# bcgsc/NanoSim

Hardware: AMD Instinct MI355X
Metric: simulated reads/sec (genome mode, mean 8 kb) (higher is better)
Workload: dtype u8

## Files before the change

nanosim_amd/csrc/nanosim_amd.hip:

```cpp
#include <hip/hip_runtime.h>
#include <hipcub/hipcub.hpp>
#include <stdio.h>
#include <stdlib.h>
#include <string.h>
#include <algorithm>
#include <chrono>
#include <atomic>
#include <condition_variable>
#include <functional>
#include <mutex>
#include <thread>
#include <type_traits>
#include <string>
#include <vector>

#include "ns_device.h"
#include "ns_materialise.h"
#include "ns_chain.h"
#include "ns_hp.h"
#include "ns_ir.h"
#include "ns_io.h"
#include "ns_pack.h"
#include "ns_cs_hist.h"
#include "ns_qual_hist.h"
// ... 950 lines not shown
                dst[L - 1 - (done + i)] = normalise_base(c);
            } else dst[done + i] = normalise_base(c);
        }
        done += end - start;
    });
    if (lane == 0) pp->ref_gpos = NS_SPLICED_BASE + off + NS_IR_PAD;
}

#ifndef NS_MAT_WAVES
#define NS_MAT_WAVES 7
#endif

__device__ __forceinline__ bool load_read_uniform(const GenArgs &A, uint64_t r, bool fastq, ns_read &rd, ns_key &key, ReadOut &ro) {
    rd = A.reads[r];
    if (rd.flags) return false;
    rd.rec_off = uni64(A.rec_off[r]);
    rd.piece_off = uni(rd.piece_off); rd.n_pieces = (uint16_t)uni(rd.n_pieces);
    rd.reversed = (uint8_t)uni(rd.reversed); rd.head = uni(rd.head); rd.tail = uni(rd.tail); rd.seq_len = uni(rd.seq_len);
    rd.attempts = uni(rd.attempts);
    key = read_key(A, r);
    key.r_lo = uni(key.r_lo); key.r_hi = uni(key.r_hi);
    ro.seq = A.records + rd.rec_off + uni(A.name_len[r]) + 2;
    ro.qual = fastq ? ro.seq + rd.seq_len + 3 : nullptr;
    ro.seq_len = rd.seq_len; ro.reversed = rd.reversed != 0; ro.uracil = A.prm.uracil != 0;
    return true;
}

#ifndef NS_MATQ_WAVES
#define NS_MATQ_WAVES 4
#endif
#ifndef NS_MATQ_MINW
#define NS_MATQ_MINW 6
#endif
__device__ __forceinline__ uint64_t hp_ev_slot(const GenArgs &A, uint64_t pos, uint32_t piece) { return (pos >> A.hp_shift) + (uint64_t)A.hp_pad * piece; }

#ifndef NS_TILE_CHUNKS_FINAL
#define NS_TILE_CHUNKS_FINAL 4u
#endif
#ifndef NS_MAT_WAVES_FINAL
#define NS_MAT_WAVES_FINAL 6
#endif
template <bool FASTQ, int MODE>
__global__ void __launch_bounds__(64, MODE == MAT_HP_FINAL ? NS_MAT_WAVES_FINAL : NS_MAT_WAVES)
k_materialise(GenArgs A, uint32_t dbg, SlowQueue sq, const uint32_t *order) {
    constexpr bool CLSOUT = FASTQ && MODE != MAT_HP_SCRATCH;
    constexpr uint32_t TC = MODE == MAT_HP_FINAL ? NS_TILE_CHUNKS_FINAL : NS_TILE_CHUNKS;
    __shared__ TileLds<TC> T;
    const uint32_t lane = threadIdx.x;
    const uint64_t slot = blockIdx.x;
    if (slot >= A.prm.n_reads) return;
    const uint64_t r = order ? (uint64_t)uni(order[slot]) : slot;
    ns_read rd; ns_key key; ReadOut ro;
    if (!load_read_uniform(A, r, false, rd, key, ro)) return;
    const uint32_t a = rd.attempts;
    tile_lds_init(T, lane);
    uint32_t *cls = nullptr;
    if constexpr (CLSOUT) cls = A.cls + cls_word0(rd.rec_off, r, cls_per_read(A.prm));
    if constexpr (MODE == MAT_HP_SCRATCH) {
        ro.seq = A.scr + uni64(A.scr_off[r]); ro.qual = nullptr; ro.reversed = false; ro.uracil = false;
        uint32_t q = 0;
        for (uint32_t pi = 0; pi < rd.n_pieces; ++pi) {
            const PieceCtx pc = load_piece_uniform(A.events, A.ref, A.pieces[rd.piece_off + pi], pi);
            materialise_piece<FASTQ, MODE, TC>(A.m, A.ref, T, ro, key, a, pc, q, lane, dbg, sq, (uint32_t)r, pi, nullptr);
            q += pc.out_len;
        }
        return;
    }
#ifdef NS_ABLATE
    if (!(dbg & 8))
#endif
    emit_head_tail(ro, key, a, rd.head, rd.tail, lane);
    uint32_t q = rd.head;
    uint64_t q_in = MODE == MAT_HP_FINAL ? uni64(A.scr_off[r]) : 0;
    for (uint32_t pi = 0; pi < rd.n_pieces; ++pi) {
        PieceCtx pc;
        if constexpr (MODE == MAT_HP_FINAL) {
            const uint32_t gp = rd.piece_off + pi;
            const ns_piece p = A.pieces[gp];
            const uint64_t eo = hp_ev_slot(A, q_in, uni(A.hp_pord[r]) + pi);
            pc.kind = uni(p.kind);
            pc.ev = A.hp_ev + eo; pc.wd = A.hp_wd + eo; pc.n_ev = pc.kind ? 0u : uni(A.hp_nev[gp]);
            pc.ref_len = uni(p.out_len); pc.out_len = pc.kind ? pc.ref_len : uni(A.hp_len[gp]);
            pc.chrom_base = (uint64_t)((uintptr_t)A.scr - (uintptr_t)A.ref.bases) + q_in; pc.chrom_len = ~0ull; pc.pos = 0;
            pc.sid = pc.kind ? NS_GAP_SEG + (pi >> 1) : (pi >> 1);
            q_in += pc.ref_len;
        } else pc = load_piece_uniform(A.events, A.ref, A.pieces[rd.piece_off + pi], pi);
        materialise_piece<FASTQ, MODE, TC>(A.m, A.ref, T, ro, key, a, pc, q, lane, dbg, sq, (uint32_t)r, pi, CLSOUT ? cls + (q >> 4) + 2u * pi : nullptr);
        q += pc.out_len;
    }
    if (A.polya) {
        const uint32_t pl = uni(A.polya[r]);
        if (pl) emit_polya(ro, q, pl, lane);
    }
}

template <bool HPF>
__global__ void __launch_bounds__(64 * NS_MATQ_WAVES, NS_MATQ_MINW) k_qualities(GenArgs A, const uint32_t *order) {
    __shared__ __align__(16) uint16_t qlut[NS_QLUT_SLOTS * 1024u];
    qual_lut_load(qlut, A.m, threadIdx.x, 64 * NS_MATQ_WAVES);
    __syncthreads();
    const uint32_t lane = threadIdx.x & 63u;
    const uint64_t slot = (uint64_t)blockIdx.x * NS_MATQ_WAVES + (threadIdx.x >> 6);
    if (slot >= A.prm.n_reads) return;
    const uint64_t r = order ? (uint64_t)uni(order[slot]) : slot;
    ns_read rd; ns_key key; ReadOut ro;
    if (!load_read_uniform(A, r, true, rd, key, ro)) return;
    const uint32_t a = rd.attempts;
    QualState Q; Q.lut = qlut;
    qualities_head_tail(A.m, Q, ro, key, a, rd.head, rd.tail, lane);
    const uint32_t *cls = A.cls + cls_word0(rd.rec_off, r, cls_per_read(A.prm));
    uint32_t q = rd.head;
    for (uint32_t pi = 0; pi < rd.n_pieces; ++pi) {
        const uint32_t gp = rd.piece_off + pi;
        const ns_piece p = A.pieces[gp];
        const uint32_t kind = uni(p.kind);
        const uint32_t out_len = (HPF && !kind) ? uni(A.hp_len[gp]) : uni(p.out_len);
        qualities_piece(A.m, Q, ro, key, a, kind ? NS_GAP_SEG + (pi >> 1) : (pi >> 1), kind, out_len, q, cls + (q >> 4) + 2u * pi, lane);
        q += out_len;
    }
    if (A.polya) {
        const uint32_t pl = uni(A.polya[r]);
        if (pl) emit_polya_quals(A.m, ro, key, a, q, pl, rd.head, rd.tail, lane);
    }
}

// ... 1205 lines not shown
        uint32_t *cnt = ctx->list_b.view<uint32_t>(), *seg_off = ctx->list_c.view<uint32_t>();
        k_dense_plan<<<dim3((unsigned)((n + 1 + 255) / 256)), dim3(256), 0, st>>>(A, cnt);
        HIPCHK(hipGetLastError());
        if (int rc = scan_sum(ctx, cnt, seg_off, n + 1)) return rc;
        const uint64_t bound = total_bases / NS_DENSE_SEG + n + 1;
        if (bound > 0x7fffffffull) return fail(ctx, NS_EINVAL, "unaligned batch too large for one launch of the record kernel (split it)");
        k_materialise_dense<<<dim3((unsigned)bound), dim3(64), 0, st>>>(A, seg_off);
        HIPCHK(hipGetLastError());
        if (fastq) {
            k_qualities<false><<<dim3((unsigned)((n + NS_MATQ_WAVES - 1) / NS_MATQ_WAVES)), dim3(64 * NS_MATQ_WAVES), 0, st>>>(A, nullptr);
            HIPCHK(hipGetLastError());
        }
        return NS_OK;
    }
    for (int round = 0;; ++round) {
        size_t cap = ctx->slow_q.cap >= 16 + sizeof(SlowTile) ? (ctx->slow_q.cap - 16) / sizeof(SlowTile) : 0;
        if (cap < n / 4 + 4096) {
            int rc = ensure(ctx, ctx->slow_q, 16 + (n / 4 + 4096) * sizeof(SlowTile));
            if (rc) return rc;
            cap = (ctx->slow_q.cap - 16) / sizeof(SlowTile);
            ctx->sq_zeroed = false;
        }
        SlowQueue sq;
        sq.count = ctx->slow_q.view<uint32_t>(); sq.items = ctx->slow_q.view<SlowTile>(16);
        sq.cap = (uint32_t)(cap > 0xffffffffull ? 0xffffffffull : cap);
        if (!(ctx->sq_zeroed && round == 0)) HIPCHK(hipMemsetAsync(sq.count, 0, 4, st));
        ctx->sq_zeroed = false;
        if (ctx->knob.dbg & 1024u) order = nullptr;
        const dim3 grid_q((unsigned)((n + NS_MATQ_WAVES - 1) / NS_MATQ_WAVES)), blk_q(64 * NS_MATQ_WAVES), grid_1((unsigned)n), blk_1(64);
        const uint32_t *order_b = (ctx->knob.dbg & 2048u) ? order : nullptr;
        if (round == 0) HIPCHK(hipEventRecord(ctx->evt[EV_RECKERNEL_BEGIN], st));
        by_fastq_mode(fastq, mode, [&](auto fq, auto md) {
            constexpr bool FQ = decltype(fq)::value; constexpr int MD = decltype(md)::value;
            k_materialise<FQ, MD><<<grid_1, blk_1, 0, st>>>(A, ctx->knob.dbg, sq, (MD == MAT_REF || (FQ && MD == MAT_HP_FINAL)) ? order_b : nullptr);
        });
        HIPCHK(hipGetLastError());
        if (round == 0) { HIPCHK(hipEventRecord(ctx->evt[EV_RECKERNEL_END], st)); ctx->rec_timed = true; }
        if (fastq && mode != MAT_HP_SCRATCH && round == 0) {
            if (mode == MAT_HP_FINAL) k_qualities<true><<<grid_q, blk_q, 0, st>>>(A, order);
            else k_qualities<false><<<grid_q, blk_q, 0, st>>>(A, order);
            HIPCHK(hipGetLastError());
        }
        uint32_t queued = 0;
        if (int rc2 = read_small(ctx, st, &queued, sq.count, 4)) return rc2;
        if (queued > sq.cap) {
            if (round >= 2) return fail(ctx, NS_ENOMEM, "slow-tile queue overflow");
            int rc = ensure(ctx, ctx->slow_q, 16 + ((size_t)queued + 4096) * sizeof(SlowTile));
            if (rc) return rc;
            continue;
        }
        if (queued) {
            const unsigned grid = queued < 16384u ? queued : 16384u;
            by_fastq_mode(fastq, mode, [&](auto fq, auto md) {
                constexpr bool FQ = decltype(fq)::value; constexpr int MD = decltype(md)::value;
                if constexpr (MD == MAT_HP_FINAL) k_materialise_slow_hpf<FQ><<<dim3(grid), dim3(64), 0, st>>>(A, sq);
                else k_materialise_slow<FQ, MD == MAT_HP_SCRATCH><<<dim3(grid), dim3(64), 0, st>>>(A, sq);
            });
            HIPCHK(hipGetLastError());
        }
        return NS_OK;
    }
}

static int hp_stage1(ns_ctx *ctx, const ns_params *prm, GenArgs &A, size_t n, uint64_t tot_pieces, unsigned long long *stats, double *ms_hp) {
    hipStream_t st = ctx->stream;
    const dim3 blk(256), grid_t((unsigned)((n + 1 + 255) / 256));
    int rc;
// ... 1858 lines not shown
```

nanosim_amd/csrc/ns_materialise.h:

```cpp
#pragma once
#include "ns_device.h"

#ifndef NS_TILE_CHUNKS
#define NS_TILE_CHUNKS 2u
#endif
#define T_EV 64u
#define NS_CLS_MIS_BIT 0x08u
#define NS_CLS_INS_BIT 0x20u
#define NS_CLS_STRIP 0xd7d7d7d7u
#define NS_QLUT_SLOTS 5u
__device__ __forceinline__ uint32_t wave_incl_scan(uint32_t v) {
    v += (uint32_t)__builtin_amdgcn_update_dpp(0, (int)v, 0x111, 0xf, 0xf, true);
    v += (uint32_t)__builtin_amdgcn_update_dpp(0, (int)v, 0x112, 0xf, 0xf, true);
    v += (uint32_t)__builtin_amdgcn_update_dpp(0, (int)v, 0x114, 0xf, 0xf, true);
    v += (uint32_t)__builtin_amdgcn_update_dpp(0, (int)v, 0x118, 0xf, 0xf, true);
    v += (uint32_t)__builtin_amdgcn_update_dpp(0, (int)v, 0x142, 0xa, 0xf, false);
    v += (uint32_t)__builtin_amdgcn_update_dpp(0, (int)v, 0x143, 0xc, 0xf, false);
    return v;
}

__device__ __forceinline__ uint32_t wave_incl_max(uint32_t v) {
    v = max(v, (uint32_t)__builtin_amdgcn_update_dpp(0, (int)v, 0x111, 0xf, 0xf, false));
    v = max(v, (uint32_t)__builtin_amdgcn_update_dpp(0, (int)v, 0x112, 0xf, 0xf, false));
    v = max(v, (uint32_t)__builtin_amdgcn_update_dpp(0, (int)v, 0x114, 0xf, 0xf, false));
    v = max(v, (uint32_t)__builtin_amdgcn_update_dpp(0, (int)v, 0x118, 0xf, 0xf, false));
    v = max(v, (uint32_t)__builtin_amdgcn_update_dpp(0, (int)v, 0x142, 0xa, 0xf, false));
    v = max(v, (uint32_t)__builtin_amdgcn_update_dpp(0, (int)v, 0x143, 0xc, 0xf, false));
    return v;
}
__device__ __forceinline__ uint32_t dpp_wave_shl1(uint32_t lane63_value, uint32_t v) {
    return (uint32_t)__builtin_amdgcn_update_dpp((int)lane63_value, (int)v, 0x130, 0xf, 0xf, false);
}

__device__ __forceinline__ uint32_t uni(uint32_t v) { return (uint32_t)__builtin_amdgcn_readfirstlane((int)v); }
__device__ __forceinline__ uint64_t uni64(uint64_t v) { return (uint64_t)uni((uint32_t)v) | (uint64_t)uni((uint32_t)(v >> 32)) << 32; }

struct ReadOut {
    uint8_t *seq;
    uint8_t *qual;
    uint32_t seq_len;
    bool reversed;
    bool uracil;
};
__device__ __forceinline__ uint64_t t_to_u8(uint64_t x) {
    const uint64_t t = x ^ 0x5454545454545454ull;
    const uint64_t z = ~(((t & 0x7f7f7f7f7f7f7f7full) + 0x7f7f7f7f7f7f7f7full) | t) & 0x8080808080808080ull;
    return x | (z >> 7);
}

typedef uint32_t ns_v4u_any __attribute__((ext_vector_type(4), aligned(1)));
__device__ __forceinline__ void store16(uint8_t *dst, uint32_t count, uint64_t lo, uint64_t hi) {
    if (count == 16) {
        ns_v4u_any x = {(uint32_t)lo, (uint32_t)(lo >> 32), (uint32_t)hi, (uint32_t)(hi >> 32)};
        __builtin_nontemporal_store(x, reinterpret_cast<ns_v4u_any *>(dst));
    } else {
        if (count & 8u) { __builtin_memcpy(dst, &lo, 8); dst += 8; lo = hi; }
        if (count & 4u) { const uint32_t w = (uint32_t)lo; __builtin_memcpy(dst, &w, 4); dst += 4; lo >>= 32; }
        if (count & 2u) { const uint16_t w = (uint16_t)lo; __builtin_memcpy(dst, &w, 2); dst += 2; lo >>= 16; }
        if (count & 1u) *dst = (uint8_t)lo;
    }
}
__device__ __forceinline__ void shift_down_bytes(uint64_t &lo, uint64_t &hi, uint32_t i0) {
    const uint32_t sh = 8 * i0;
    if (sh == 0) return;
    if (sh < 64) { lo = (lo >> sh) | (hi << (64 - sh)); hi >>= sh; }
    else { lo = hi >> (sh - 64); hi = 0; }
}
__device__ __forceinline__ void reverse_bytes(uint64_t &lo, uint64_t &hi, uint32_t count) {
    uint64_t rlo = __builtin_bswap64(hi), rhi = __builtin_bswap64(lo);
    uint32_t s = 8 * (16 - count);
    if (s == 0) { lo = rlo; hi = rhi; }
    else if (s < 64) { lo = (rlo >> s) | (rhi << (64 - s)); hi = rhi >> s; }
    else { lo = rhi >> (s - 64); hi = 0; }
}
__device__ __forceinline__ uint64_t complement8(uint64_t x) {
    return x ^ 0x1515151515151515ull ^ (((x >> 1) & 0x0101010101010101ull) * 0x11ull);
}
__device__ __forceinline__ void store_chunk(const ReadOut &ro, uint32_t q0, uint32_t count, uint64_t lo, uint64_t hi,
                                            uint64_t qlo, uint64_t qhi) {
    uint32_t o0 = q0;
    if (ro.reversed) {
        lo = complement8(lo); hi = complement8(hi);
        reverse_bytes(lo, hi, count);
        o0 = ro.seq_len - q0 - count;
    }
    if (ro.uracil) { lo = t_to_u8(lo); hi = t_to_u8(hi); }
    store16(ro.seq + o0, count, lo, hi);
    if (ro.qual) {
        qlo += 0x2121212121212121ull; qhi += 0x2121212121212121ull;
        if (ro.reversed) reverse_bytes(qlo, qhi, count);
        store16(ro.qual + o0, count, qlo, qhi);
    }
}
struct PendingChunk { uint64_t lo, hi, qlo, qhi; uint32_t o0, count; };
__device__ __forceinline__ PendingChunk prep_chunk(const ReadOut &ro, uint32_t q0, uint32_t count, uint64_t lo, uint64_t hi,
                                                   uint64_t qlo, uint64_t qhi) {
    PendingChunk p; p.count = count; p.o0 = q0;
    if (ro.reversed) {
        if (count == 16) {
            const uint32_t w0 = (uint32_t)lo, w1 = (uint32_t)(lo >> 32), w2 = (uint32_t)hi, w3 = (uint32_t)(hi >> 32);
            const uint32_t c0 = __builtin_amdgcn_perm(0x43000041u, 0x47005400u, w0 & 0x07070707u), c1 = __builtin_amdgcn_perm(0x43000041u, 0x47005400u, w1 & 0x07070707u);
            const uint32_t c2 = __builtin_amdgcn_perm(0x43000041u, 0x47005400u, w2 & 0x07070707u), c3 = __builtin_amdgcn_perm(0x43000041u, 0x47005400u, w3 & 0x07070707u);
            const uint32_t r0 = __builtin_amdgcn_perm(0u, c3, 0x00010203u), r1 = __builtin_amdgcn_perm(0u, c2, 0x00010203u);
            const uint32_t r2 = __builtin_amdgcn_perm(0u, c1, 0x00010203u), r3 = __builtin_amdgcn_perm(0u, c0, 0x00010203u);
            lo = (uint64_t)r0 | (uint64_t)r1 << 32; hi = (uint64_t)r2 | (uint64_t)r3 << 32;
        } else {
            lo = complement8(lo); hi = complement8(hi);
            reverse_bytes(lo, hi, count);
        }
        p.o0 = ro.seq_len - q0 - count;
    }
    if (ro.uracil) { lo = t_to_u8(lo); hi = t_to_u8(hi); }
    p.lo = lo; p.hi = hi; p.qlo = 0; p.qhi = 0;
    if (ro.qual) {
        qlo += 0x2121212121212121ull; qhi += 0x2121212121212121ull;
        if (ro.reversed) reverse_bytes(qlo, qhi, count);
        p.qlo = qlo; p.qhi = qhi;
    }
    return p;
}
__device__ __forceinline__ void flush_chunk(const ReadOut &ro, PendingChunk &p) {
    if (!p.count) return;
    store16(ro.seq + p.o0, p.count, p.lo, p.hi);
    if (ro.qual) store16(ro.qual + p.o0, p.count, p.qlo, p.qhi);
    p.count = 0;
}
__device__ __forceinline__ void put_byte(uint64_t &lo, uint64_t &hi, uint32_t i, uint32_t b) {
    if (i < 8) lo |= (uint64_t)b << (8 * i); else hi |= (uint64_t)b << (8 * (i - 8));
}

struct QualDraw {
    uint32_t blk; u32x4 w;
};
__device__ __forceinline__ uint32_t qual_draw(QualDraw &qd, const DevModel &m, int cls, const ns_key &key, uint32_t stream,
                                              uint32_t seg, uint32_t attempt, uint32_t mpos) {
    if ((mpos >> 3) != qd.blk) { qd.blk = mpos >> 3; qd.w = ns_draw(key, stream, seg, attempt, qd.blk, 0); }
    uint32_t h = (ns_word(qd.w, (mpos & 7) >> 1) >> (16 * (mpos & 1))) & 0xffffu;
    return qual_value_lut(m.qual_thr + cls * NS_QUAL_LEVELS, m.qual_lut + cls * 1024, h);
}

__device__ __forceinline__ uint32_t ins_letters4(uint32_t word, uint32_t k) {
    const uint32_t x = (word >> (8u * k)) & 0xffu, t = (x | x << 12) & 0x000f000fu;
    return __builtin_amdgcn_perm(0u, 0x47435441u, (t | t << 6) & 0x03030303u);
}

__device__ inline void emit_head_tail(const ReadOut &ro, const ns_key &key, uint32_t a, uint32_t head, uint32_t tail, uint32_t lane) {
    const bool is_tail = lane >= 32;
    const uint32_t len = is_tail ? tail : head, stream = is_tail ? ST_TAIL : ST_HEAD;
    const uint32_t q_start = is_tail ? ro.seq_len - tail : 0u;
    for (uint32_t i0 = (lane & 31u) * 16; i0 < len; i0 += 32 * 16) {
        const uint32_t count = min(16u, len - i0);
        u32x4 w = ns_draw(key, stream, 0, a, i0 >> 6, 0);
        const uint32_t word = ns_word(w, (i0 >> 4) & 3);
        uint32_t l4[4];
#pragma unroll
        for (uint32_t k = 0; k < 4; ++k) l4[k] = ins_letters4(word, k);
        const uint64_t lo = (uint64_t)l4[0] | (uint64_t)l4[1] << 32, hi = (uint64_t)l4[2] | (uint64_t)l4[3] << 32;
        store_chunk(ro, q_start + i0, count, lo, hi, 0, 0);
    }
// ... 80 lines not shown
            uint32_t x = c.cur_pos + d;
            uint8_t cur = resolve_base(ref_base_at(ref, pc, x), key, pc.sid, attempt, x);
            return mis_letter(cur, key, pc.sid, attempt, c.j - 1, d);
        }
        cls = NS_Q_INS;
        return ins_letter(key, pc.sid, attempt, c.j - 1, d);
    }
    cls = NS_Q_MATCH;
    uint32_t x = c.cur_rp + (d - c.cur_pl);
    return resolve_base(ref_base_at(ref, pc, x), key, pc.sid, attempt, x);
}
NS_DEV PieceCtx load_piece(const ns_event *events, const DevRef &ref, const ns_piece &p, uint32_t pi) {
    PieceCtx pc;
    pc.ev = events + p.ev_off; pc.wd = nullptr; pc.n_ev = p.n_ev; pc.out_len = p.out_len; pc.ref_len = p.ref_len;
    pc.chrom_base = ref.chrom_off[p.chrom];
    pc.chrom_len = ref.chrom_off[p.chrom + 1] - pc.chrom_base;
    if (p.ref_gpos >= NS_SPLICED_BASE) {
        pc.chrom_base = (uint64_t)((uintptr_t)ref.spliced - (uintptr_t)ref.bases) + (p.ref_gpos - NS_SPLICED_BASE) - p.pos;
        pc.chrom_len = ~0ull;
    }
    pc.pos = p.pos; pc.kind = p.kind;
    pc.sid = p.kind ? NS_GAP_SEG + (pi >> 1) : (pi >> 1);
    return pc;
}
__device__ __forceinline__ PieceCtx load_piece_uniform(const ns_event *events, const DevRef &ref, const ns_piece &p, uint32_t pi) {
    PieceCtx pc;
    const uint64_t eo = uni64(p.ev_off);
    pc.ev = events + eo; pc.wd = nullptr; pc.n_ev = uni(p.n_ev); pc.out_len = uni(p.out_len); pc.ref_len = uni(p.ref_len);
    const uint32_t chrom = uni(p.chrom);
    pc.chrom_base = uni64(ref.chrom_off[chrom]);
    pc.chrom_len = uni64(ref.chrom_off[chrom + 1]) - pc.chrom_base;
    pc.pos = uni(p.pos); pc.kind = uni(p.kind);
    const uint64_t gpos = uni64(p.ref_gpos);
    if (gpos >= NS_SPLICED_BASE) {
        pc.chrom_base = (uint64_t)((uintptr_t)ref.spliced - (uintptr_t)ref.bases) + (gpos - NS_SPLICED_BASE) - pc.pos;
        pc.chrom_len = ~0ull;
    }
    pc.sid = pc.kind ? NS_GAP_SEG + (pi >> 1) : (pi >> 1);
    return pc;
}
template <bool CLS_BITS = false>
__device__ inline void slow_piece_range(const DevModel &m, const DevRef &ref, const ReadOut &ro, const ns_key &key, uint32_t a,
                                        const PieceCtx &pc, uint32_t pq, uint32_t m_lo, uint32_t m_hi, uint32_t lane) {
    for (uint32_t m0 = m_lo + lane * 16; m0 < m_hi; m0 += 64 * 16) {
        const uint32_t count = min(16u, m_hi - m0);
        Cursor cur;
        cursor_seek(cur, pc, m0);
        uint64_t lo = 0, hi = 0, qlo = 0, qhi = 0;
        QualDraw qd; qd.blk = 0xffffffffu;
        for (uint32_t i = 0; i < count; ++i) {
            int cls;
            uint32_t b = piece_byte(ref, pc, cur, m0 + i, key, a, cls);
            if constexpr (CLS_BITS) b |= cls == NS_Q_MIS ? NS_CLS_MIS_BIT : cls == NS_Q_INS ? NS_CLS_INS_BIT : 0u;
            put_byte(lo, hi, i, b);
            if (ro.qual) put_byte(qlo, qhi, i, qual_draw(qd, m, pc.kind ? NS_Q_UNMAPPED : cls, key, ST_QUAL, pc.sid, a, m0 + i));
        }
        store_chunk(ro, pq + m0, count, lo, hi, qlo, qhi);
    }
}

__device__ __forceinline__ void wave_sync() {
    __builtin_amdgcn_fence(__ATOMIC_ACQ_REL, "wavefront");
    __builtin_amdgcn_wave_barrier();
}

typedef __attribute__((address_space(3))) volatile uint8_t *LdsBytes;
typedef __attribute__((address_space(3))) volatile uint32_t *LdsWords;
// ... 240 lines not shown
__device__ __forceinline__ void lds_or64(uint8_t *p, uint64_t v) {
    __hip_atomic_fetch_or(reinterpret_cast<unsigned long long *>(p), (unsigned long long)v, __ATOMIC_RELAXED, __HIP_MEMORY_SCOPE_WAVEFRONT);
}

template <int MODE>
__device__ __forceinline__ uint32_t event_word(const PieceCtx &pc, const ns_key &key, uint32_t a, uint32_t j) {
    if constexpr (MODE == MAT_HP_FINAL) return pc.wd[j];
    else { const u32x4 w = ns_draw(key, ST_SUB, pc.sid, a, j >> 2, 0); return ns_word(w, j & 3u); }
}
template <uint32_t TC>
struct __align__(16) TileLds {
    static constexpr uint32_t T_OUT_ = 1024u * TC;
    uint32_t mlut[17][4];
    uint2 ent[T_EV + 1];
    uint32_t eos[T_EV + 1];
    uint32_t hist[64 * TC];
    __align__(16) uint8_t out[1024u * TC + 16 + 64];
};
template <uint32_t TC>
__device__ __forceinline__ void tile_lds_init(TileLds<TC> &T, uint32_t lane) {
    for (uint32_t c = lane * 16; c < 1024u * TC + 16 + 64; c += 64 * 16) *reinterpret_cast<uint4 *>(&T.out[c]) = make_uint4(0, 0, 0, 0);
    if (lane < 17) {
#pragma unroll
        for (uint32_t k = 0; k < 4; ++k)
            T.mlut[lane][k] = lane <= 4 * k ? 0xffffffffu : lane >= 4 * k + 4 ? 0u : 0xffffffffu << (8 * (lane - 4 * k));
    }
}
#ifdef NS_ABLATE
#define NS_DBG(bit) (dbg & (bit))
#else
#define NS_DBG(bit) false
#endif
__device__ __forceinline__ uint32_t and_andn(uint32_t a, uint32_t b, uint32_t c) { return __builtin_amdgcn_bitop3_b32(a, b, c, 0x40); }
template <bool FASTQ, int MODE, uint32_t TC>
__device__ inline void materialise_piece(const DevModel &m, const DevRef &ref, TileLds<TC> &T, const ReadOut &ro, const ns_key &key,
                                         uint32_t a, const PieceCtx &pc, uint32_t pq, uint32_t lane, uint32_t dbg, const SlowQueue &sq,
                                         uint32_t read_idx, uint32_t piece_idx, uint32_t *__restrict__ cls) {
    constexpr bool CLSOUT = FASTQ && MODE != MAT_HP_SCRATCH;
    constexpr bool HPF = MODE == MAT_HP_FINAL;
    constexpr uint32_t T_OUT_ = 1024u * TC;
    uint32_t jb = 0;
    uint32_t L0_out = 0, L0_rp = 0, L0_pt = 3u << 12, L0_wd = 0, L0_j = 0;
    const uint8_t *seg0 = ref.bases + pc.chrom_base + pc.pos;
    const bool wraps = !HPF && pc.pos + pc.ref_len > pc.chrom_len;
    const uint32_t wrap_at = wraps ? (uint32_t)(pc.chrom_len - pc.pos) : 0xffffffffu;
    const uint32_t phi = ro.reversed ? ((uint32_t)(uintptr_t)ro.seq + ro.seq_len - pq) & 15u : (0u - ((uint32_t)(uintptr_t)ro.seq + pq)) & 15u;
    ns_event e_pre; e_pre.pos = 0; e_pre.info = 0; uint32_t w_pre = 0;
    if (lane < pc.n_ev) e_pre = pc.ev[lane];
    auto cached_word = [&](uint32_t j0) -> uint32_t { if (NS_DBG(64u)) return 0u; const uint32_t j = j0 + lane; return event_word<MODE>(pc, key, a, j < pc.n_ev ? j : 0u); };
    w_pre = cached_word(0u);
    uint32_t cls_carry = 0;
    for (uint32_t M0 = 0; M0 < pc.out_len;) {
        const uint32_t A0 = M0 - ((M0 - phi) & 15u);
        uint32_t M1 = min(A0 + T_OUT_, pc.out_len);
        const ns_event e = e_pre;
        const uint32_t e_wd = w_pre;
        const bool valid = jb + lane < pc.n_ev;
        const uint32_t os = ev_out_start(e), len = ns_ev_len(e.info), ty = ns_ev_type(e.info);
        const uint32_t e_pt = ev_letters(ty, len) | ty << 12, e_rp = ev_resume(e.pos, ty, len);
        if (jb + 63 < pc.n_ev) {
            const uint32_t os63 = (uint32_t)__builtin_amdgcn_readlane((int)os, 63);
            if (os63 < M1) {
                const uint32_t cut = A0 + ((os63 - A0) & ~15u);
                M1 = (int32_t)(cut - M0) > 0 ? cut : os63;
            }
        }
        const bool take = valid && os < M1;
        const uint32_t cnt = (uint32_t)__popcll(__ballot(take));
        if (M1 <= M0) {
            cls_carry = 0;
            M1 = min(M0 + T_OUT_, pc.out_len);
            uint32_t j2 = jb;
            while (j2 < pc.n_ev && ev_out_start(pc.ev[j2]) < M1) ++j2;
            slow_queue_push(sq, lane, SlowTile{read_idx, piece_idx, M0, M1});
            if (j2 > jb) {
                const ns_event le = pc.ev[j2 - 1];
                const uint32_t ll = ns_ev_len(le.info), lt = ns_ev_type(le.info);
                L0_out = uni(ev_out_start(le)); L0_pt = uni(ev_letters(lt, ll) | lt << 12); L0_rp = uni(ev_resume(le.pos, lt, ll));
                L0_wd = uni(event_word<MODE>(pc, key, a, j2 - 1)); L0_j = uni(j2 - 1);
            }
            jb = uni(j2); M0 = M1;
            e_pre.pos = 0; e_pre.info = 0; w_pre = 0;
            if (jb + lane < pc.n_ev) e_pre = pc.ev[jb + lane];
            w_pre = cached_word(jb);
            continue;
        }
        const uint32_t nc = (M1 - A0 + 15u) >> 4;
        const uint32_t ekey = take ? (os <= M0 ? 0u : (os - A0 + 15u) >> 4) : 0xffffffffu;
        const uint32_t s1 = os + (e_pt & 0xfffu), y1 = e_rp - s1;
        {
            const uint32_t s0 = L0_out + (L0_pt & 0xfffu);
            T.ent[0] = make_uint2(s0, L0_rp - s0);
            if (take) T.ent[1 + lane] = make_uint2(s1, y1);
            T.eos[lane] = take ? os : 0xffffffffu;
        }
#pragma unroll
        for (uint32_t t = 0; t < TC; ++t) T.hist[64 * t + lane] = 0;
        const uint32_t jb_next = jb + cnt;
        e_pre.pos = 0; e_pre.info = 0; w_pre = 0;
        if (M1 < pc.out_len && jb_next + lane < pc.n_ev) e_pre = pc.ev[jb_next + lane];
        if (M1 < pc.out_len) w_pre = cached_word(jb_next);
        wave_sync();
        const uint32_t os_next = dpp_wave_shl1(0xffffffffu, take ? os : 0xffffffffu);
        {
            const uint32_t c_next = dpp_wave_shl1(0xffffffffu, ekey);
            if (ekey < 64 * TC && ekey != c_next) T.hist[ekey] = lane + 1u;
        }
        uint32_t osl = L0_out, ptl = L0_pt, rpl = L0_rp, wdl = L0_wd, jl = L0_j;
        if (cnt) {
            osl = (uint32_t)__builtin_amdgcn_readlane((int)os, (int)(cnt - 1));
            ptl = (uint32_t)__builtin_amdgcn_readlane((int)e_pt, (int)(cnt - 1));
            rpl = (uint32_t)__builtin_amdgcn_readlane((int)e_rp, (int)(cnt - 1));
            wdl = (uint32_t)__builtin_amdgcn_readlane((int)e_wd, (int)(cnt - 1));
            jl = jb + cnt - 1;
        }
        const uint8_t *tb = seg0 - 32;
        bool fast = true;
        if (wraps) {
            const uint32_t pl0 = L0_pt & 0xfffu, ty0 = L0_pt >> 12, d0 = M0 - L0_out;
            const uint32_t x0 = (d0 < pl0 && ty0 == NS_INS) ? L0_rp : L0_rp + d0 - pl0;
            const uint32_t pll = ptl & 0xfffu, dl = M1 - osl;
            uint32_t x1 = dl <= pll ? rpl : rpl + (dl - pll);
            if (x1 < x0) x1 = x0;
            if (x0 >= wrap_at) tb -= pc.chrom_len;
            else if (x1 > wrap_at) fast = false;
        }
        if (!fast) {
            cls_carry = 0;
            slow_queue_push(sq, lane, SlowTile{read_idx, piece_idx, M0, M1});
            L0_out = osl; L0_rp = rpl; L0_pt = ptl; L0_wd = wdl; L0_j = jl;
            jb = jb_next; M0 = M1;
            wave_sync();
            continue;
        }
        wave_sync();
        uint4 f[TC]; uint32_t fi[TC], fy[TC];
        {
            uint32_t scan_base = 0;
#pragma unroll
            for (uint32_t t = 0; t < TC; ++t) {
                const uint32_t ci = 64 * t + lane;
                const uint32_t incl = max(scan_base, wave_incl_max(T.hist[ci]));
                scan_base = (uint32_t)__builtin_amdgcn_readlane((int)incl, 63);
                f[t] = make_uint4(0, 0, 0, 0); fi[t] = 16u | 16u << 8; fy[t] = 0;
                if (ci < nc && !NS_DBG(1u) && !NS_DBG(256u)) {
                    const uint32_t cs = A0 + 16u * ci, p = ci == 0 ? M0 : cs;
                    const uint2 E = T.ent[incl];
                    const uint32_t nx = T.eos[incl];
                    const uint32_t st = max(p, E.x), en = min(nx, min(cs + 16u, M1));
                    if ((int32_t)(en - st) > 0) {
                        fi[t] = (st - cs) | (en - cs) << 8; fy[t] = E.y;
                        __builtin_memcpy(&f[t], tb + (E.y + cs + 32u), 16);
                    }
                }
            }
        }
        uint4 fe = make_uint4(0, 0, 0, 0); uint32_t ei0 = 16, ei1 = 16, eoc = 0;
        if (take && !NS_DBG(1u) && !NS_DBG(128u)) {
            const uint32_t c = (s1 - A0) >> 4, ecs = A0 + 16u * c;
            const uint32_t en = min(os_next, min(ecs + 16u, M1));
            if ((int32_t)(en - s1) > 0 && ekey > c) {
                eoc = 16u * c; ei0 = s1 - ecs; ei1 = en - ecs;
                __builtin_memcpy(&fe, tb + (y1 + ecs + 32u), 16);
            }
        }
        if (!NS_DBG(2u)) {
            const bool cont = lane == 63 && L0_out + (L0_pt & 0xfffu) > M0;
            const uint32_t b_os = cont ? L0_out : os, b_pt = cont ? L0_pt : e_pt, b_rp = cont ? L0_rp : e_rp;
            const uint32_t b_j = cont ? L0_j : jb + lane;
            uint32_t frac = cont ? L0_wd : e_wd;
            const uint32_t b_pl = b_pt & 0xfffu, b_ty = b_pt >> 12;
            const bool on = (take || cont) && b_pl;
            const uint32_t xs = b_rp - b_pl;
            const bool mis = b_ty == NS_MIS;
            bool fast_l = on && b_pl <= 8 && b_os >= M0 && b_os + b_pl <= M1 && !wraps;
            uint2 cur8 = make_uint2(0x41414141u, 0x41414141u);
            if (fast_l && mis) __builtin_memcpy(&cur8, seg0 + xs, 8);
            const uint64_t keep = b_pl >= 8u ? ~0ull : ~(~0ull << (8u * b_pl));
            if constexpr (!HPF) fast_l = fast_l && !(((uint64_t)cur8.x | (uint64_t)cur8.y << 32) & keep & 0x8080808080808080ull);
            if (fast_l) {
                uint32_t f3 = frac, L2[2];
#pragma unroll
                for (uint32_t g = 0; g < 2; ++g) {
                    const uint32_t cur4 = g ? cur8.y : cur8.x;
                    const uint32_t ins4 = ins_letters4(frac, g);
                    const uint32_t d0 = next_digit3(f3), d1 = next_digit3(f3), d2 = next_digit3(f3), d3 = next_digit3(f3);
                    const uint32_t d4 = d0 | d1 << 8 | d2 << 16 | d3 << 24;
                    const uint32_t vv = (cur4 >> 1) & 0x03030303u;
                    const uint32_t rank4 = (vv & 0x01010101u) << 1 | ((vv >> 1) & 0x01010101u);
                    const uint32_t ge = ((d4 | 0x80808080u) - rank4) & 0x80808080u;
                    const uint32_t mis4 = __builtin_amdgcn_perm(0u, 0x47435441u, d4 + (ge >> 7));
                    uint32_t letters = mis ? mis4 : ins4;
                    if constexpr (FASTQ) {
                        uint32_t cls4 = mis ? 0x01010101u * NS_CLS_MIS_BIT : 0x01010101u * NS_CLS_INS_BIT;
                        if constexpr (HPF) {
                            if (mis) cls4 = (frac & 1u) ? NS_CLS_MIS_BIT : (cur4 & (NS_CLS_MIS_BIT | NS_CLS_INS_BIT));
                            else if (g == 0 && (frac >> 31)) cls4 = (cls4 & ~0xffu) | NS_CLS_MIS_BIT;
                        }
                        letters |= cls4;
                    }
                    L2[g] = letters;
                }
                const uint64_t v = ((uint64_t)L2[0] | (uint64_t)L2[1] << 32) & keep;
                const uint32_t o = b_os - A0, sh = 8u * (o & 3u);
                const uint64_t lo64 = v << sh;
                const uint32_t top = (uint32_t)(((v >> 32) << sh) >> 32);
                uint8_t *w = &T.out[o & ~3u];
                lds_or32(w, (uint32_t)lo64); lds_or32(w + 4, (uint32_t)(lo64 >> 32)); lds_or32(w + 8, top);
            }
            if (on && !fast_l) {
                const uint32_t i_lo = b_os < M0 ? M0 - b_os : 0u;
                const uint32_t i_hi = min(b_pl, M1 - b_os);
                const uint32_t word0 = frac;
                for (uint32_t i = 0; i < i_hi; ++i) {
                    if (i && !(i & 15)) frac = payload_word(key, pc.sid, a, b_j, i >> 4);
                    uint32_t b;
                    if (b_ty == NS_INS) {
                        b = bases_atcg((frac >> (2 * (i & 15))) & 3u);
                        if constexpr (FASTQ) b |= (HPF && i == 0 && (word0 >> 31)) ? NS_CLS_MIS_BIT : NS_CLS_INS_BIT;
                    } else {
                        const uint32_t x = xs + i;
                        const uint32_t src = ref_base_at(ref, pc, x);
                        if constexpr (HPF) {
                            b = mis_from_digit(src & ~(NS_CLS_MIS_BIT | NS_CLS_INS_BIT), next_digit3(frac));
                            if constexpr (FASTQ) b |= (word0 & 1u) ? NS_CLS_MIS_BIT : (src & (NS_CLS_MIS_BIT | NS_CLS_INS_BIT));
                        } else {
                            b = mis_from_digit(resolve_base(src, key, pc.sid, a, x), next_digit3(frac));
                            if constexpr (FASTQ) b |= NS_CLS_MIS_BIT;
                        }
                    }
                    if (i >= i_lo) T.out[b_os + i - A0] = (uint8_t)b;
                }
            }
        }
        if (cnt && ei0 < 16u && !NS_DBG(32u)) {
            const uint4 m0 = *reinterpret_cast<const uint4 *>(&T.mlut[ei0][0]), m1 = *reinterpret_cast<const uint4 *>(&T.mlut[ei1][0]);
            uint32_t a0 = and_andn(fe.x, m0.x, m1.x), a1 = and_andn(fe.y, m0.y, m1.y), a2 = and_andn(fe.z, m0.z, m1.z), a3 = and_andn(fe.w, m0.w, m1.w);
            if constexpr (!HPF) {
                if ((a0 | a1 | a2 | a3) & 0x80808080u) resolve16(a0, a1, a2, a3, 0xffffu, A0 + eoc + y1, key, pc.sid, a);
            }
            lds_or64(&T.out[eoc], (uint64_t)a0 | (uint64_t)a1 << 32);
            lds_or64(&T.out[eoc + 8], (uint64_t)a2 | (uint64_t)a3 << 32);
        }
        wave_sync();
#pragma unroll
        for (uint32_t t = 0; t < TC; ++t) {
            const uint32_t ci = 64 * t + lane;
            const uint32_t c0 = A0 + 16 * ci;
            const uint32_t lo_m = ci == 0 ? M0 : c0, hi_m = min(c0 + 16, M1);
            const bool active = (int32_t)(hi_m - lo_m) > 0 && !NS_DBG(1u);
            uint32_t cw = 0;
            if (active) {
                const uint4 v = *reinterpret_cast<const uint4 *>(&T.out[16 * ci]);
                *reinterpret_cast<uint4 *>(&T.out[16 * ci]) = make_uint4(0, 0, 0, 0);
                const uint32_t i0 = fi[t] & 0xffu, i1 = fi[t] >> 8;
                const uint4 m0 = *reinterpret_cast<const uint4 *>(&T.mlut[i0][0]), m1 = *reinterpret_cast<const uint4 *>(&T.mlut[i1][0]);
                uint32_t a0 = and_andn(f[t].x, m0.x, m1.x), a1 = and_andn(f[t].y, m0.y, m1.y), a2 = and_andn(f[t].z, m0.z, m1.z), a3 = and_andn(f[t].w, m0.w, m1.w);
                if constexpr (!HPF) {
                    if ((a0 | a1 | a2 | a3) & 0x80808080u) resolve16(a0, a1, a2, a3, 0xffffu, c0 + fy[t], key, pc.sid, a);
                }
                if (NS_DBG(512u)) { a0 = a1 = a2 = a3 = 0x41414141u; }
                uint32_t r0 = v.x | a0, r1 = v.y | a1, r2 = v.z | a2, r3 = v.w | a3;
                uint32_t s0 = lo_m - c0, count = hi_m - lo_m;
                if constexpr (CLSOUT) {
                    cw = cls_pack16(r0, r1, r2, r3);
                    if (ci == 0) cw |= cls_carry;
                    if (!pc.kind) cls[(c0 + ((0u - phi) & 15u)) >> 4] = cw;
                    r0 &= NS_CLS_STRIP; r1 &= NS_CLS_STRIP; r2 &= NS_CLS_STRIP; r3 &= NS_CLS_STRIP;
                }
                uint64_t lo = (uint64_t)r0 | (uint64_t)r1 << 32, hi = (uint64_t)r2 | (uint64_t)r3 << 32;
                if (s0) {
                    const uint32_t sh = 8 * s0;
                    if (sh < 64) { lo = (lo >> sh) | (hi << (64 - sh)); hi >>= sh; }
                    else { lo = hi >> (sh - 64); hi = 0; }
                }
                if (!NS_DBG(16u)) { PendingChunk pd = prep_chunk(ro, pq + lo_m, count, lo, hi, 0, 0); flush_chunk(ro, pd); }
            }
            if constexpr (CLSOUT) {
                const uint32_t cl = (M1 - 1u - A0) >> 4;
                if (t == (cl >> 6)) cls_carry = (M1 < pc.out_len && ((M1 - A0) & 15u)) ? (uint32_t)__builtin_amdgcn_readlane((int)cw, (int)(cl & 63u)) : 0u;
            }
        }
        L0_out = osl; L0_rp = rpl; L0_pt = ptl; L0_wd = wdl; L0_j = jl;
        jb = jb_next; M0 = M1;
        wave_sync();
    }
}

__device__ __forceinline__ void quals16(const QualState &Q, const DevModel &m, const ns_key &key, uint32_t stream, uint32_t sid, uint32_t a,
                                        uint32_t j, const uint32_t cs[4], uint64_t &qlo, uint64_t &qhi) {
    const u32x4 k1 = ns_draw(key, stream, sid, a, 2u * j, 0), k2 = ns_draw(key, stream, sid, a, 2u * j + 1u, 0);
    const uint32_t D[8] = {k1.x, k1.y, k1.z, k1.w, k2.x, k2.y, k2.z, k2.w};
    qual_lookup16(Q, m, D, cs, qlo, qhi);
}
__device__ inline void qualities_piece(const DevModel &m, const QualState &Q, const ReadOut &ro, const ns_key &key, uint32_t a, uint32_t sid,
                                       uint32_t kind, uint32_t out_len, uint32_t pq, const uint32_t *__restrict__ cls, uint32_t lane) {
    const uint32_t phi = ro.reversed ? ((uint32_t)(uintptr_t)ro.seq + ro.seq_len - pq) & 15u : (0u - ((uint32_t)(uintptr_t)ro.seq + pq)) & 15u;
    const uint32_t g2 = 2u * ((0u - phi) & 15u);
    const uint32_t nchunks = (out_len + 15u) >> 4;
    uint32_t wl = 0, wh = 0;
    if (!kind && lane < nchunks) { wl = cls[lane]; wh = cls[lane + 1u]; }
    for (uint32_t j = lane; j < nchunks; j += 64) {
        const uint32_t w = __builtin_amdgcn_alignbit(wh, wl, g2);
        if (!kind && j + 64u < nchunks) { wl = cls[j + 64u]; wh = cls[j + 65u]; }
        uint32_t cs[4];
        if (kind) cs[0] = cs[1] = cs[2] = cs[3] = 0x08080808u * (uint32_t)NS_Q_UNMAPPED;
        else { cs[0] = cls_unpack4(w, 0); cs[1] = cls_unpack4(w, 1); cs[2] = cls_unpack4(w, 2); cs[3] = cls_unpack4(w, 3); }
        uint64_t qlo, qhi;
        quals16(Q, m, key, ST_QUAL, sid, a, j, cs, qlo, qhi);
// ... 20 lines not shown
```

Measured before the change: 135.2 million.

## Specialise materialise kernel on strand and uracil, read cold args from kernarg segment

Templates materialise_piece on reverse-strand and uracil flags so the per-chunk output path loses runtime branches and the dead quality handling. Rarely used values (slow queue, order, chromosome lengths) are re-read on demand from the kernel-argument segment through a Cold helper instead of being held in registers, which aims to cut SGPR/VGPR pressure. Wrap checks become scalar tests on wrap_at and the spliced-base test compares only the high word. The cost is more template instantiations, larger code, and extra scalar loads on cold paths.

```diff
diff --git a/nanosim_amd/csrc/nanosim_amd.hip b/nanosim_amd/csrc/nanosim_amd.hip
--- a/nanosim_amd/csrc/nanosim_amd.hip
+++ b/nanosim_amd/csrc/nanosim_amd.hip
@@ -1006,7 +1006,8 @@
 #ifndef NS_MATQ_MINW
 #define NS_MATQ_MINW 6
 #endif
-__device__ __forceinline__ uint64_t hp_ev_slot(const GenArgs &A, uint64_t pos, uint32_t piece) { return (pos >> A.hp_shift) + (uint64_t)A.hp_pad * piece; }
+__device__ __forceinline__ uint64_t hp_ev_slot(uint32_t hp_shift, uint32_t hp_pad, uint64_t pos, uint32_t piece) { return (pos >> hp_shift) + (uint64_t)hp_pad * piece; }
+__device__ __forceinline__ uint64_t hp_ev_slot(const GenArgs &A, uint64_t pos, uint32_t piece) { return hp_ev_slot(A.hp_shift, A.hp_pad, pos, piece); }
 
 #ifndef NS_TILE_CHUNKS_FINAL
 #define NS_TILE_CHUNKS_FINAL 4u
@@ -1014,57 +1015,92 @@
 #ifndef NS_MAT_WAVES_FINAL
 #define NS_MAT_WAVES_FINAL 6
 #endif
-template <bool FASTQ, int MODE>
+struct MatArgs { GenArgs A; SlowQueue sq; const uint32_t *order; uint32_t dbg; };
+typedef const __attribute__((address_space(4))) MatArgs *MatArgsPtr;
+__device__ __forceinline__ MatArgsPtr mat_args_now() {
+    MatArgsPtr p = (MatArgsPtr)__builtin_amdgcn_kernarg_segment_ptr();
+    asm volatile("" : "+s"(p));
+    return p;
+}
+struct MatCold {
+    uint32_t gp, pi;
+    __device__ __forceinline__ void push(uint32_t lane, uint32_t m0, uint32_t m1) const {
+        const uint32_t *order = mat_args_now()->order;
+        const uint32_t r = order ? uni(order[blockIdx.x]) : blockIdx.x;
+        const MatArgsPtr K = mat_args_now();
+        SlowQueue sq; sq.items = K->sq.items; sq.count = K->sq.count; sq.cap = K->sq.cap;
+        slow_queue_push(sq, lane, SlowTile{r, pi, m0, m1});
+    }
+    __device__ __forceinline__ uint64_t chrom_len() const {
+        const MatArgsPtr K = mat_args_now();
+        const ns_piece *pieces = K->A.pieces;
+        const uint64_t *off = K->A.ref.chrom_off;
+        const uint32_t chrom = uni(pieces[gp].chrom);
+        return uni64(off[chrom + 1]) - uni64(off[chrom]);
+    }
+};
+
+template <bool FASTQ, int MODE, uint32_t TC, bool URACIL>
+__device__ __forceinline__ uint32_t materialise_pieces(const GenArgs &A, TileLds<TC> &T, const ReadOut &ro, const ns_key &key, const ns_read &rd,
+                                                       uint64_t r, uint32_t q, uint32_t lane, uint32_t dbg) {
+    constexpr bool CLSOUT = FASTQ && MODE != MAT_HP_SCRATCH;
+    const uint32_t a = rd.attempts;
+    uint32_t *cls = nullptr;
+    if constexpr (CLSOUT) cls = A.cls + cls_word0(rd.rec_off, r, cls_per_read(A.prm));
+    uint64_t q_in = MODE == MAT_HP_FINAL ? uni64(A.scr_off[r]) : 0;
+    for (uint32_t pi = 0; pi < rd.n_pieces; ++pi) {
+        PieceCtx pc;
+        const uint32_t gp = rd.piece_off + pi;
+        if constexpr (MODE == MAT_HP_FINAL) {
+            const MatArgsPtr K = mat_args_now();
+            const ns_piece *pieces = K->A.pieces;
+            const uint32_t *hp_pord = K->A.hp_pord, *hp_nev = K->A.hp_nev, *hp_len = K->A.hp_len;
+            const ns_piece p = pieces[gp];
+            const uint64_t eo = hp_ev_slot(K->A.hp_shift, K->A.hp_pad, q_in, uni(hp_pord[r]) + pi);
+            pc.kind = uni(p.kind);
+            pc.ev = K->A.hp_ev + eo; pc.wd = K->A.hp_wd + eo; pc.n_ev = pc.kind ? 0u : uni(hp_nev[gp]);
+            pc.ref_len = uni(p.out_len); pc.out_len = pc.kind ? pc.ref_len : uni(hp_len[gp]);
+            pc.chrom_base = (uint64_t)((uintptr_t)K->A.scr - (uintptr_t)K->A.ref.bases) + q_in; pc.chrom_len = ~0ull; pc.pos = 0;
+            pc.sid = pc.kind ? NS_GAP_SEG + (pi >> 1) : (pi >> 1);
+            q_in += pc.ref_len;
+        } else pc = load_piece_uniform(A.events, A.ref, A.pieces[gp], pi);
+        uint32_t *const pcls = CLSOUT ? cls + (q >> 4) + 2u * pi : nullptr;
+        if (ro.reversed) materialise_piece<FASTQ, MODE, TC, true, URACIL>(A.ref, T, PieceOut<true>(ro, q), key, a, pc, lane, dbg, MatCold{gp, pi}, pcls);
+        else materialise_piece<FASTQ, MODE, TC, false, URACIL>(A.ref, T, PieceOut<false>(ro, q), key, a, pc, lane, dbg, MatCold{gp, pi}, pcls);
+        q += pc.out_len;
+    }
+    return q;
+}
+
+template <bool FASTQ, int MODE, bool URACIL>
 __global__ void __launch_bounds__(64, MODE == MAT_HP_FINAL ? NS_MAT_WAVES_FINAL : NS_MAT_WAVES)
-k_materialise(GenArgs A, uint32_t dbg, SlowQueue sq, const uint32_t *order) {
-    constexpr bool CLSOUT = FASTQ && MODE != MAT_HP_SCRATCH;
+k_materialise(MatArgs K) {
+    static_assert(std::is_trivially_copyable<MatArgs>::value && offsetof(MatArgs, A) == 0, "MatArgs is read back from the kernel-argument segment as it was passed");
     constexpr uint32_t TC = MODE == MAT_HP_FINAL ? NS_TILE_CHUNKS_FINAL : NS_TILE_CHUNKS;
     __shared__ TileLds<TC> T;
+    const GenArgs &A = K.A;
     const uint32_t lane = threadIdx.x;
     const uint64_t slot = blockIdx.x;
     if (slot >= A.prm.n_reads) return;
-    const uint64_t r = order ? (uint64_t)uni(order[slot]) : slot;
+    const uint64_t r = K.order ? (uint64_t)uni(K.order[slot]) : slot;
     ns_read rd; ns_key key; ReadOut ro;
     if (!load_read_uniform(A, r, false, rd, key, ro)) return;
-    const uint32_t a = rd.attempts;
     tile_lds_init(T, lane);
-    uint32_t *cls = nullptr;
-    if constexpr (CLSOUT) cls = A.cls + cls_word0(rd.rec_off, r, cls_per_read(A.prm));
     if constexpr (MODE == MAT_HP_SCRATCH) {
+        static_assert(MODE != MAT_HP_SCRATCH || !URACIL, "the scratch pass of -k writes T");
         ro.seq = A.scr + uni64(A.scr_off[r]); ro.qual = nullptr; ro.reversed = false; ro.uracil = false;
-        uint32_t q = 0;
-        for (uint32_t pi = 0; pi < rd.n_pieces; ++pi) {
-            const PieceCtx pc = load_piece_uniform(A.events, A.ref, A.pieces[rd.piece_off + pi], pi);
-            materialise_piece<FASTQ, MODE, TC>(A.m, A.ref, T, ro, key, a, pc, q, lane, dbg, sq, (uint32_t)r, pi, nullptr);
-            q += pc.out_len;
-        }
-        return;
-    }
+        materialise_pieces<FASTQ, MODE, TC, false>(A, T, ro, key, rd, r, 0u, lane, K.dbg);
+    } else {
+        ro.uracil = URACIL;
 #ifdef NS_ABLATE
-    if (!(dbg & 8))
+        if (!(K.dbg & 8))
 #endif
-    emit_head_tail(ro, key, a, rd.head, rd.tail, lane);
-    uint32_t q = rd.head;
-    uint64_t q_in = MODE == MAT_HP_FINAL ? uni64(A.scr_off[r]) : 0;
-    for (uint32_t pi = 0; pi < rd.n_pieces; ++pi) {
-        PieceCtx pc;
-        if constexpr (MODE == MAT_HP_FINAL) {
-            const uint32_t gp = rd.piece_off + pi;
-            const ns_piece p = A.pieces[gp];
-            const uint64_t eo = hp_ev_slot(A, q_in, uni(A.hp_pord[r]) + pi);
-            pc.kind = uni(p.kind);
-            pc.ev = A.hp_ev + eo; pc.wd = A.hp_wd + eo; pc.n_ev = pc.kind ? 0u : uni(A.hp_nev[gp]);
-            pc.ref_len = uni(p.out_len); pc.out_len = pc.kind ? pc.ref_len : uni(A.hp_len[gp]);
-            pc.chrom_base = (uint64_t)((uintptr_t)A.scr - (uintptr_t)A.ref.bases) + q_in; pc.chrom_len = ~0ull; pc.pos = 0;
-            pc.sid = pc.kind ? NS_GAP_SEG + (pi >> 1) : (pi >> 1);
-            q_in += pc.ref_len;
-        } else pc = load_piece_uniform(A.events, A.ref, A.pieces[rd.piece_off + pi], pi);
-        materialise_piece<FASTQ, MODE, TC>(A.m, A.ref, T, ro, key, a, pc, q, lane, dbg, sq, (uint32_t)r, pi, CLSOUT ? cls + (q >> 4) + 2u * pi : nullptr);
-        q += pc.out_len;
-    }
-    if (A.polya) {
-        const uint32_t pl = uni(A.polya[r]);
-        if (pl) emit_polya(ro, q, pl, lane);
+        emit_head_tail(ro, key, rd.attempts, rd.head, rd.tail, lane);
+        const uint32_t q = materialise_pieces<FASTQ, MODE, TC, URACIL>(A, T, ro, key, rd, r, rd.head, lane, K.dbg);
+        if (A.polya) {
+            const uint32_t pl = uni(A.polya[r]);
+            if (pl) emit_polya(ro, q, pl, lane);
+        }
     }
 }
 
@@ -2336,7 +2372,9 @@
         if (round == 0) HIPCHK(hipEventRecord(ctx->evt[EV_RECKERNEL_BEGIN], st));
         by_fastq_mode(fastq, mode, [&](auto fq, auto md) {
             constexpr bool FQ = decltype(fq)::value; constexpr int MD = decltype(md)::value;
-            k_materialise<FQ, MD><<<grid_1, blk_1, 0, st>>>(A, ctx->knob.dbg, sq, (MD == MAT_REF || (FQ && MD == MAT_HP_FINAL)) ? order_b : nullptr);
+            const MatArgs K{A, sq, (MD == MAT_REF || (FQ && MD == MAT_HP_FINAL)) ? order_b : nullptr, ctx->knob.dbg};
+            if (MD != MAT_HP_SCRATCH && A.prm.uracil) k_materialise<FQ, MD, MD != MAT_HP_SCRATCH><<<grid_1, blk_1, 0, st>>>(K);
+            else k_materialise<FQ, MD, false><<<grid_1, blk_1, 0, st>>>(K);
         });
         HIPCHK(hipGetLastError());
         if (round == 0) { HIPCHK(hipEventRecord(ctx->evt[EV_RECKERNEL_END], st)); ctx->rec_timed = true; }
diff --git a/nanosim_amd/csrc/ns_materialise.h b/nanosim_amd/csrc/ns_materialise.h
--- a/nanosim_amd/csrc/ns_materialise.h
+++ b/nanosim_amd/csrc/ns_materialise.h
@@ -35,6 +35,8 @@
 __device__ __forceinline__ uint32_t uni(uint32_t v) { return (uint32_t)__builtin_amdgcn_readfirstlane((int)v); }
 __device__ __forceinline__ uint64_t uni64(uint64_t v) { return (uint64_t)uni((uint32_t)v) | (uint64_t)uni((uint32_t)(v >> 32)) << 32; }
 
+__device__ __forceinline__ uint32_t here(uint32_t v) { asm volatile("" : "+s"(v)); return v; }
+
 struct ReadOut {
     uint8_t *seq;
     uint8_t *qual;
@@ -92,11 +94,9 @@
         store16(ro.qual + o0, count, qlo, qhi);
     }
 }
-struct PendingChunk { uint64_t lo, hi, qlo, qhi; uint32_t o0, count; };
-__device__ __forceinline__ PendingChunk prep_chunk(const ReadOut &ro, uint32_t q0, uint32_t count, uint64_t lo, uint64_t hi,
-                                                   uint64_t qlo, uint64_t qhi) {
-    PendingChunk p; p.count = count; p.o0 = q0;
-    if (ro.reversed) {
+template <bool REV, bool URACIL>
+__device__ __forceinline__ void emit_chunk(uint8_t *dst, uint32_t count, uint64_t lo, uint64_t hi) {
+    if constexpr (REV) {
         if (count == 16) {
             const uint32_t w0 = (uint32_t)lo, w1 = (uint32_t)(lo >> 32), w2 = (uint32_t)hi, w3 = (uint32_t)(hi >> 32);
             const uint32_t c0 = __builtin_amdgcn_perm(0x43000041u, 0x47005400u, w0 & 0x07070707u), c1 = __builtin_amdgcn_perm(0x43000041u, 0x47005400u, w1 & 0x07070707u);
@@ -108,23 +108,17 @@
             lo = complement8(lo); hi = complement8(hi);
             reverse_bytes(lo, hi, count);
         }
-        p.o0 = ro.seq_len - q0 - count;
-    }
-    if (ro.uracil) { lo = t_to_u8(lo); hi = t_to_u8(hi); }
-    p.lo = lo; p.hi = hi; p.qlo = 0; p.qhi = 0;
-    if (ro.qual) {
-        qlo += 0x2121212121212121ull; qhi += 0x2121212121212121ull;
-        if (ro.reversed) reverse_bytes(qlo, qhi, count);
-        p.qlo = qlo; p.qhi = qhi;
-    }
-    return p;
-}
-__device__ __forceinline__ void flush_chunk(const ReadOut &ro, PendingChunk &p) {
-    if (!p.count) return;
-    store16(ro.seq + p.o0, p.count, p.lo, p.hi);
-    if (ro.qual) store16(ro.qual + p.o0, p.count, p.qlo, p.qhi);
-    p.count = 0;
-}
+    }
+    if constexpr (URACIL) { lo = t_to_u8(lo); hi = t_to_u8(hi); }
+    store16(dst, count, lo, hi);
+}
+template <bool REV>
+struct PieceOut {
+    uint8_t *base;
+    __device__ __forceinline__ PieceOut(const ReadOut &ro, uint32_t pq) : base(REV ? ro.seq + (ro.seq_len - pq) : ro.seq + pq) {}
+    __device__ __forceinline__ uint8_t *at(uint32_t lo_m, uint32_t hi_m) const { return REV ? base - hi_m : base + lo_m; }
+    __device__ __forceinline__ uint32_t phi() const { return (REV ? (uint32_t)(uintptr_t)base : 0u - (uint32_t)(uintptr_t)base) & 15u; }
+};
 __device__ __forceinline__ void put_byte(uint64_t &lo, uint64_t &hi, uint32_t i, uint32_t b) {
     if (i < 8) lo |= (uint64_t)b << (8 * i); else hi |= (uint64_t)b << (8 * (i - 8));
 }
@@ -271,7 +265,8 @@
     pc.chrom_len = uni64(ref.chrom_off[chrom + 1]) - pc.chrom_base;
     pc.pos = uni(p.pos); pc.kind = uni(p.kind);
     const uint64_t gpos = uni64(p.ref_gpos);
-    if (gpos >= NS_SPLICED_BASE) {
+    static_assert((uint32_t)NS_SPLICED_BASE == 0, "the test below reads the high word only");
+    if (here((uint32_t)(gpos >> 32)) >= (uint32_t)(NS_SPLICED_BASE >> 32)) {
         pc.chrom_base = (uint64_t)((uintptr_t)ref.spliced - (uintptr_t)ref.bases) + (gpos - NS_SPLICED_BASE) - pc.pos;
         pc.chrom_len = ~0ull;
     }
@@ -578,19 +573,20 @@
 #define NS_DBG(bit) false
 #endif
 __device__ __forceinline__ uint32_t and_andn(uint32_t a, uint32_t b, uint32_t c) { return __builtin_amdgcn_bitop3_b32(a, b, c, 0x40); }
-template <bool FASTQ, int MODE, uint32_t TC>
-__device__ inline void materialise_piece(const DevModel &m, const DevRef &ref, TileLds<TC> &T, const ReadOut &ro, const ns_key &key,
-                                         uint32_t a, const PieceCtx &pc, uint32_t pq, uint32_t lane, uint32_t dbg, const SlowQueue &sq,
-                                         uint32_t read_idx, uint32_t piece_idx, uint32_t *__restrict__ cls) {
+template <bool FASTQ, int MODE, uint32_t TC, bool REV, bool URACIL, typename Cold>
+__device__ inline void materialise_piece(const DevRef &ref, TileLds<TC> &T, const PieceOut<REV> out, const ns_key &key,
+                                         uint32_t a, const PieceCtx &pc, uint32_t lane, uint32_t dbg, const Cold &cold,
+                                         uint32_t *__restrict__ cls) {
     constexpr bool CLSOUT = FASTQ && MODE != MAT_HP_SCRATCH;
     constexpr bool HPF = MODE == MAT_HP_FINAL;
     constexpr uint32_t T_OUT_ = 1024u * TC;
     uint32_t jb = 0;
     uint32_t L0_out = 0, L0_rp = 0, L0_pt = 3u << 12, L0_wd = 0, L0_j = 0;
     const uint8_t *seg0 = ref.bases + pc.chrom_base + pc.pos;
-    const bool wraps = !HPF && pc.pos + pc.ref_len > pc.chrom_len;
-    const uint32_t wrap_at = wraps ? (uint32_t)(pc.chrom_len - pc.pos) : 0xffffffffu;
-    const uint32_t phi = ro.reversed ? ((uint32_t)(uintptr_t)ro.seq + ro.seq_len - pq) & 15u : (0u - ((uint32_t)(uintptr_t)ro.seq + pq)) & 15u;
+    const uint32_t wrap_at = (!HPF && pc.pos + pc.ref_len > pc.chrom_len) ? (uint32_t)(pc.chrom_len - pc.pos) : 0xffffffffu;
+    const uint32_t fast_pl = wrap_at != 0xffffffffu ? 0u : 8u;
+    auto base_at = [&](uint32_t x) -> uint32_t { const uint8_t *s = seg0; if (!HPF && x >= wrap_at) s -= cold.chrom_len(); return s[x]; };
+    const uint32_t phi = out.phi();
     ns_event e_pre; e_pre.pos = 0; e_pre.info = 0; uint32_t w_pre = 0;
     if (lane < pc.n_ev) e_pre = pc.ev[lane];
     auto cached_word = [&](uint32_t j0) -> uint32_t { if (NS_DBG(64u)) return 0u; const uint32_t j = j0 + lane; return event_word<MODE>(pc, key, a, j < pc.n_ev ? j : 0u); };
@@ -618,7 +614,7 @@
             M1 = min(M0 + T_OUT_, pc.out_len);
             uint32_t j2 = jb;
             while (j2 < pc.n_ev && ev_out_start(pc.ev[j2]) < M1) ++j2;
-            slow_queue_push(sq, lane, SlowTile{read_idx, piece_idx, M0, M1});
+            cold.push(lane, M0, M1);
             if (j2 > jb) {
                 const ns_event le = pc.ev[j2 - 1];
                 const uint32_t ll = ns_ev_len(le.info), lt = ns_ev_type(le.info);
@@ -662,18 +658,18 @@
         }
         const uint8_t *tb = seg0 - 32;
         bool fast = true;
-        if (wraps) {
+        if (!HPF && here(wrap_at) != 0xffffffffu) {
             const uint32_t pl0 = L0_pt & 0xfffu, ty0 = L0_pt >> 12, d0 = M0 - L0_out;
             const uint32_t x0 = (d0 < pl0 && ty0 == NS_INS) ? L0_rp : L0_rp + d0 - pl0;
             const uint32_t pll = ptl & 0xfffu, dl = M1 - osl;
             uint32_t x1 = dl <= pll ? rpl : rpl + (dl - pll);
             if (x1 < x0) x1 = x0;
-            if (x0 >= wrap_at) tb -= pc.chrom_len;
+            if (x0 >= wrap_at) tb -= cold.chrom_len();
             else if (x1 > wrap_at) fast = false;
         }
         if (!fast) {
             cls_carry = 0;
-            slow_queue_push(sq, lane, SlowTile{read_idx, piece_idx, M0, M1});
+            cold.push(lane, M0, M1);
             L0_out = osl; L0_rp = rpl; L0_pt = ptl; L0_wd = wdl; L0_j = jl;
             jb = jb_next; M0 = M1;
             wave_sync();
@@ -719,7 +715,7 @@
             const bool on = (take || cont) && b_pl;
             const uint32_t xs = b_rp - b_pl;
             const bool mis = b_ty == NS_MIS;
-            bool fast_l = on && b_pl <= 8 && b_os >= M0 && b_os + b_pl <= M1 && !wraps;
+            bool fast_l = on && b_pl <= fast_pl && b_os >= M0 && b_os + b_pl <= M1;
             uint2 cur8 = make_uint2(0x41414141u, 0x41414141u);
             if (fast_l && mis) __builtin_memcpy(&cur8, seg0 + xs, 8);
             const uint64_t keep = b_pl >= 8u ? ~0ull : ~(~0ull << (8u * b_pl));
@@ -766,7 +762,7 @@
                         if constexpr (FASTQ) b |= (HPF && i == 0 && (word0 >> 31)) ? NS_CLS_MIS_BIT : NS_CLS_INS_BIT;
                     } else {
                         const uint32_t x = xs + i;
-                        const uint32_t src = ref_base_at(ref, pc, x);
+                        const uint32_t src = base_at(x);
                         if constexpr (HPF) {
                             b = mis_from_digit(src & ~(NS_CLS_MIS_BIT | NS_CLS_INS_BIT), next_digit3(frac));
                             if constexpr (FASTQ) b |= (word0 & 1u) ? NS_CLS_MIS_BIT : (src & (NS_CLS_MIS_BIT | NS_CLS_INS_BIT));
@@ -820,7 +816,7 @@
                     if (sh < 64) { lo = (lo >> sh) | (hi << (64 - sh)); hi >>= sh; }
                     else { lo = hi >> (sh - 64); hi = 0; }
                 }
-                if (!NS_DBG(16u)) { PendingChunk pd = prep_chunk(ro, pq + lo_m, count, lo, hi, 0, 0); flush_chunk(ro, pd); }
+                if (!NS_DBG(16u)) emit_chunk<REV, URACIL>(out.at(lo_m, hi_m), count, lo, hi);
             }
             if constexpr (CLSOUT) {
                 const uint32_t cl = (M1 - 1u - A0) >> 4;
```

Result: faster. 142.9 million (median of 6 runs) (+5.7%).
